# davidmilligan/MLVFS

Hardware: AMD Instinct MI355X
Metric: Mpix/s, 3584x1320 14-bit unpack+badpix+cs5x5+stripes (fused, stream resident in HBM) (higher is better)
Workload: dtype u16/int32

## Files before the change

### mlvfs_amd/csrc/k_frame_p.hip

```cpp
#include "frame_plan.h"
#include "k_stream_dev.h"

namespace mlv {

constexpr int P_WAIT_MIN = 1, P_WAIT_MAX = 15;
template <bool SPREAD_>
struct __align__(16) SmemP {
    static constexpr bool SPREAD = SPREAD_;
    uint16_t raw[2 * RH][2 * TCW];
    uint32_t pk[PH][PW];
    int ge[RH][TCW];
    uint16_t t16[MLV_T16_N + (SPREAD_ ? 64 : 0)];
    uint32_t has_patch[PMAP_WORDS];
    uint32_t xchg[3][XCHG_WORDS];
    int unc[2];
    int low[2];
    int dim[2];
    int next_tile, next_end;
    int walk[5];
    int2 carry_at[256];
    uint4 carry_spare;
};

struct PGroup {
    mlv_pk16 s[4][5];
    mlv_pk16 p0[10], p1[10];
    mlv_pk16 q[6];
};
struct PNext { mlv_pk16 s0[5], s2[5], p0[10], q[6]; };

__device__ __forceinline__ mlv_pk16 as_pk(uint32_t v) { return __builtin_bit_cast(mlv_pk16, v); }
__device__ __forceinline__ uint32_t as_u(mlv_pk16 v) { return __builtin_bit_cast(uint32_t, v); }

__device__ __forceinline__ void pchain_group(const uint32_t (*pk)[PW], int row_top, int col_left, PGroup &g)
{
    mlv_pk16 col[4][5];
#pragma unroll
    for (int r = 0; r < 5; r++) {
        const uint4 v = *(const uint4 *)&pk[row_top + r][col_left];
        col[0][r] = as_pk(v.x); col[1][r] = as_pk(v.y); col[2][r] = as_pk(v.z); col[3][r] = as_pk(v.w);
    }
#pragma unroll
    for (int c = 0; c < 4; c++) mlv_sort5(col[c], g.s[c]);
    mlv_merge55(g.s[0], g.s[1], g.p0);
    mlv_merge55(g.s[2], g.s[3], g.p1);
}
__device__ __forceinline__ void pchain_fetch_lists(const PGroup &g, PNext &n)
{
#pragma unroll
    for (int i = 0; i < 5; i++) { n.s0[i] = dpp_next(g.s[0][i]); n.s2[i] = dpp_next(g.s[2][i]); }
#pragma unroll
    for (int i = 0; i < 10; i++) n.p0[i] = dpp_next(g.p0[i]);
}
__device__ __forceinline__ void pchain_fetch_window(const PGroup &g, PNext &n)
{
#pragma unroll
    for (int i = 0; i < 6; i++) n.q[i] = dpp_next(g.q[i]);
}
__device__ __forceinline__ void pchain_publish(const PGroup &g, uint32_t *x)
{
    uint4 *o = (uint4 *)x;
    o[0] = make_uint4(as_u(g.s[0][0]), as_u(g.s[0][1]), as_u(g.s[0][2]), as_u(g.s[0][3]));
    o[1] = make_uint4(as_u(g.s[0][4]), as_u(g.s[2][0]), as_u(g.s[2][1]), as_u(g.s[2][2]));
    o[2] = make_uint4(as_u(g.s[2][3]), as_u(g.s[2][4]), as_u(g.p0[0]), as_u(g.p0[1]));
    o[3] = make_uint4(as_u(g.p0[2]), as_u(g.p0[3]), as_u(g.p0[4]), as_u(g.p0[5]));
    o[4] = make_uint4(as_u(g.p0[6]), as_u(g.p0[7]), as_u(g.p0[8]), as_u(g.p0[9]));
    o[5] = make_uint4(as_u(g.q[0]), as_u(g.q[1]), as_u(g.q[2]), as_u(g.q[3]));
    *(uint2 *)&o[6] = make_uint2(as_u(g.q[4]), as_u(g.q[5]));
}
__device__ __forceinline__ void pchain_collect_lists(const uint32_t *x, PNext &n)
{
    const uint4 *o = (const uint4 *)x;
    const uint4 a0 = o[0], a1 = o[1], a2 = o[2], a3 = o[3], a4 = o[4];
    n.s0[0] = as_pk(a0.x); n.s0[1] = as_pk(a0.y); n.s0[2] = as_pk(a0.z); n.s0[3] = as_pk(a0.w); n.s0[4] = as_pk(a1.x);
    n.s2[0] = as_pk(a1.y); n.s2[1] = as_pk(a1.z); n.s2[2] = as_pk(a1.w); n.s2[3] = as_pk(a2.x); n.s2[4] = as_pk(a2.y);
    n.p0[0] = as_pk(a2.z); n.p0[1] = as_pk(a2.w); n.p0[2] = as_pk(a3.x); n.p0[3] = as_pk(a3.y); n.p0[4] = as_pk(a3.z);
    n.p0[5] = as_pk(a3.w); n.p0[6] = as_pk(a4.x); n.p0[7] = as_pk(a4.y); n.p0[8] = as_pk(a4.z); n.p0[9] = as_pk(a4.w);
}
__device__ __forceinline__ void pchain_collect_window(const uint32_t *x, PNext &n)
{
    const uint4 a5 = *(const uint4 *)(x + 20);
    const uint2 a6 = *(const uint2 *)(x + 24);
    n.q[0] = as_pk(a5.x); n.q[1] = as_pk(a5.y); n.q[2] = as_pk(a5.z); n.q[3] = as_pk(a5.w); n.q[4] = as_pk(a6.x); n.q[5] = as_pk(a6.y);
}
__device__ __forceinline__ void pchain_finish(const PGroup &g, const PNext &n, mlv_pk16 (&o)[STRIP])
{
    mlv_pk16 q1[6], t[1];
    mlv_quad_mid6(g.p1, n.p0, q1);
    mlv_final6of11(g.q, n.s0, t);  o[0] = t[0];
    mlv_final6of11(q1, g.s[1], t); o[1] = t[0];
    mlv_final6of11(q1, n.s2, t);   o[2] = t[0];
    mlv_final6of11(n.q, g.s[3], t); o[3] = t[0];
}
__device__ __forceinline__ bool pk_uncertain(const mlv_pk16 (&o)[STRIP])
{
    typedef unsigned short upk16 __attribute__((ext_vector_type(2)));
    const upk16 off = { 32769, 32769 }, two = { 2, 2 };
    upk16 m = __builtin_bit_cast(upk16, o[0]) + off;
#pragma unroll
    for (int c = 1; c < STRIP; c++) m = __builtin_elementwise_min(m, (upk16)(__builtin_bit_cast(upk16, o[c]) + off));
    return __builtin_bit_cast(uint32_t, __builtin_elementwise_min(m, two)) != 0x00020002u;
}

__device__ __forceinline__ uint32_t add3_u32(uint32_t a, uint32_t b, uint32_t c)
{
    uint32_t r;
    asm("v_add3_u32 %0, %1, %2, %3" : "=v"(r) : "v"(a), "v"(b), "v"(c));
    return r;
}
template <int NC, bool SPREAD>
__device__ __forceinline__ void cell_multi_pk_fast(const uint32_t *p0, const uint32_t *p1, int black, const uint16_t *t, int ref_r, int ref_b,
                                                   int (&ge)[NC], uint32_t (&pk)[NC])
{
    uint32_t fb[4 * NC], tv[4 * NC];
    const float fmagic = 8388608.0f + (float)black;
#pragma unroll
    for (int c = 0; c < NC; c++) {
        const uint32_t px[4] = { p0[2 * c], p0[2 * c + 1], p1[2 * c], p1[2 * c + 1] };
#pragma unroll
        for (int i = 0; i < 4; i++) fb[4 * c + i] = __float_as_uint(__uint_as_float(px[i] | 0x4B000000u) - fmagic);
    }
#pragma unroll
    for (int i = 0; i < 4 * NC; i++) tv[i] = *(const uint16_t *)((const char *)t + t16_offset<SPREAD>(fb[i]));
    uint32_t exr[NC], exb[NC], exg[NC];
#pragma unroll
    for (int c = 0; c < NC; c++) { exr[c] = fb[4 * c] >> 8; exb[c] = fb[4 * c + 3] >> 8; exg[c] = (fb[4 * c + 1] + fb[4 * c + 2]) >> 8; }
#pragma unroll
    for (int c = 0; c < NC; c += 2) {
        asm volatile("" :: "v"(exr[c]), "v"(exb[c]), "v"(exg[c]), "v"(exr[c + 1]), "v"(exb[c + 1]), "v"(exg[c + 1]));
    }
#pragma unroll
    for (int i = 0; i < 4 * NC; i += 8) {
        asm volatile("" :: "v"(tv[i]), "v"(tv[i + 1]), "v"(tv[i + 2]), "v"(tv[i + 3]), "v"(tv[i + 4]), "v"(tv[i + 5]), "v"(tv[i + 6]), "v"(tv[i + 7]));
    }
    uint32_t nref_r = 0u - (uint32_t)ref_r, nref_b = 0u - (uint32_t)ref_b;
    asm("" : "+v"(nref_r), "+v"(nref_b));
#pragma unroll
    for (int c = 0; c < NC; c++) {
        const uint32_t gb = add3_u32(exg[c], tv[4 * c + 1], tv[4 * c + 2]) >> 1;
        ge[c] = (int)(gb - (127u << 15));
        uint32_t ngr = nref_r - gb, ngb = nref_b - gb;
        pk[c] = as_u(__builtin_amdgcn_cvt_pk_i16((int)add3_u32(exr[c], tv[4 * c + 0], ngr), (int)add3_u32(exb[c], tv[4 * c + 3], ngb)));
    }
}

template <int NC>
__device__ __forceinline__ void cell_multi_pk_tab(const uint32_t *p0, const uint32_t *p1, uint32_t koff, const int *tab, int ref_r, int ref_b,
                                                  int (&ge)[NC], uint32_t (&pk)[NC])
{
    uint32_t ev[4 * NC];
#pragma unroll
    for (int c = 0; c < NC; c++) {
        const uint32_t px[4] = { p0[2 * c], p0[2 * c + 1], p1[2 * c], p1[2 * c + 1] };
#pragma unroll
        for (int i = 0; i < 4; i++) ev[4 * c + i] = *(const uint32_t *)((const char *)tab + ((px[i] << 2) + koff));
    }
#pragma unroll
    for (int i = 0; i < 4 * NC; i += 8) {
        asm volatile("" :: "v"(ev[i]), "v"(ev[i + 1]), "v"(ev[i + 2]), "v"(ev[i + 3]), "v"(ev[i + 4]), "v"(ev[i + 5]), "v"(ev[i + 6]), "v"(ev[i + 7]));
    }
    uint32_t nref_r = 1u - (uint32_t)ref_r, nref_b = 1u - (uint32_t)ref_b;
    asm("" : "+v"(nref_r), "+v"(nref_b));
#pragma unroll
    for (int c = 0; c < NC; c++) {
        const uint32_t gb = (ev[4 * c + 1] + ev[4 * c + 2]) >> 1;
        ge[c] = (int)gb;
        const uint32_t ng = ~gb;
        pk[c] = as_u(__builtin_amdgcn_cvt_pk_i16((int)add3_u32(ev[4 * c + 0], nref_r, ng), (int)add3_u32(ev[4 * c + 3], nref_b, ng)));
    }
}
template <int NC>
__device__ __forceinline__ void cell_multi_pk_tab_dark(const uint32_t *p0, const uint32_t *p1, uint32_t koff, const int *tab, int ref_r, int ref_b,
                                                       int (&ge)[NC], uint32_t (&pk)[NC])
{
    int ev[4 * NC];
#pragma unroll
    for (int c = 0; c < NC; c++) {
        const uint32_t px[4] = { p0[2 * c], p0[2 * c + 1], p1[2 * c], p1[2 * c + 1] };
#pragma unroll
        for (int i = 0; i < 4; i++) ev[4 * c + i] = *(const int *)((const char *)tab + max((int)((px[i] << 2) + koff), 0));
    }
#pragma unroll
    for (int i = 0; i < 4 * NC; i += 8) {
        asm volatile("" :: "v"(ev[i]), "v"(ev[i + 1]), "v"(ev[i + 2]), "v"(ev[i + 3]), "v"(ev[i + 4]), "v"(ev[i + 5]), "v"(ev[i + 6]), "v"(ev[i + 7]));
    }
#pragma unroll
    for (int c = 0; c < NC; c++) {
        ge[c] = half_trunc(wadd(ev[4 * c + 1], ev[4 * c + 2]));
        const int dr = wsub(ev[4 * c + 0], ge[c]), db = wsub(ev[4 * c + 3], ge[c]);
        pk[c] = as_u(__builtin_amdgcn_cvt_pk_i16(__builtin_elementwise_sub_sat(dr, ref_r), __builtin_elementwise_sub_sat(db, ref_b)));
    }
}

template <class SM>
__device__ __forceinline__ void emit_item_p(SM &sm, int black, bool dark, bool slow, int ref_r, int ref_b, int p, int lk, bool edge,
                                            const uint32_t (&p0)[8], const uint32_t (&p1)[8])
{
    const int jj = p - HC;
    const bool keep = !edge && jj >= 0;
    int ge[4];
    uint32_t pk[4];
    if (!dark) cell_multi_pk_fast<4, SM::SPREAD>(p0, p1, black, sm.t16, ref_r, ref_b, ge, pk);
    else {
        int dr[4], db[4];
#pragma unroll
        for (int c = 0; c < 4; c += 2) {
            int g2[2], r2[2], b2[2];
            if (!slow) cell_multi_ev_dark<2, SM::SPREAD>(p0 + 2 * c, p1 + 2 * c, black, sm.t16, g2, r2, b2);
            else cell_pair_ev<SM::SPREAD>(p0 + 2 * c, p1 + 2 * c, black, sm.t16, true, g2, r2, b2);
            ge[c] = g2[0]; ge[c + 1] = g2[1]; dr[c] = r2[0]; dr[c + 1] = r2[1]; db[c] = b2[0]; db[c + 1] = b2[1];
        }
#pragma unroll
        for (int c = 0; c < 4; c++)
            pk[c] = as_u(__builtin_amdgcn_cvt_pk_i16(__builtin_elementwise_sub_sat(dr[c], ref_r), __builtin_elementwise_sub_sat(db[c], ref_b)));
    }
    const int ca = edge ? PW - HC : HC + 4 * lk, cb = edge ? 0 : ca + 2;
    const uint32_t prow = __umul24((uint32_t)p, (uint32_t)(PW * 4));
    char *ppk = (char *)&sm.pk[0][0] + prow;
    *(uint2 *)(ppk + 4 * ca) = make_uint2(pk[0], pk[1]);
    *(uint2 *)(ppk + 4 * cb) = make_uint2(pk[2], pk[3]);
    if (keep) {
        *(int4 *)&sm.ge[jj][4 * lk] = make_int4(ge[0], ge[1], ge[2], ge[3]);
        *(uint4 *)&sm.raw[2 * jj][8 * lk] = make_uint4(p0[0] | (p0[1] << 16), p0[2] | (p0[3] << 16), p0[4] | (p0[5] << 16), p0[6] | (p0[7] << 16));
        *(uint4 *)&sm.raw[2 * jj + 1][8 * lk] = make_uint4(p1[0] | (p1[1] << 16), p1[2] | (p1[3] << 16), p1[4] | (p1[5] << 16), p1[6] | (p1[7] << 16));
    }
}

template <bool PACKED, int VEC, bool SPREAD>
__global__ __launch_bounds__(256, 4) void k_frame_p(const FrameArgs a)
{
    static_assert(VEC != 0, "rows of whole 8-pixel groups");
    constexpr int METHOD = 5;
    using Smem = SmemP<SPREAD>;
    __shared__ Smem sm;
    constexpr int BPP = bpp_of(PACKED, VEC);
    constexpr int NEW0 = 2 * HC;
    const int tid = threadIdx.x;

    load_t16_rel<SPREAD>(sm.t16, cold_args()->t16, tid);
    {
        constexpr int C_PL = 2 * HC * PW * 4 / 16, C_RAW = 2 * HC * 2 * TCW * 2 / 16, C_GE = HC * TCW * 4 / 16, C_ALL = C_PL + C_RAW + C_GE;
        static_assert(C_ALL <= 256, "one 16-byte piece per thread");
        int to = (int)offsetof(Smem, carry_spare), delta = 0;
        if (tid < C_PL) { to = (int)offsetof(Smem, pk) + 16 * tid; delta = TCH * PW * 4; }
        else if (tid < C_PL + C_RAW) { to = (int)offsetof(Smem, raw) + 16 * (tid - C_PL); delta = 2 * TCH * 2 * TCW * 2; }
        else if (tid < C_ALL) { to = (int)offsetof(Smem, ge) + 16 * (tid - C_PL - C_RAW); delta = TCH * TCW * 4; }
        sm.carry_at[tid] = make_int2(to + delta, to);
    }
    const int tiles_per_frame = a.tiles_x * a.tiles_y;
    const bool pmap_ok = tiles_per_frame <= PMAP_WORDS * 32;
    int band_end;
    {
        KArgs ka = cold_args();
        if (ka->patch && pmap_ok) {
            for (int i = tid; i < PMAP_WORDS; i += 256) sm.has_patch[i] = 0;
            __syncthreads();
            const int *toff = ka->tile_off;
            for (int i = tid; i < tiles_per_frame; i += 256)
                if (toff[i + 1] != toff[i]) atomicOr(&sm.has_patch[i >> 5], 1u << (i & 31));
        }
        const int total = tiles_per_frame * ka->nframes;
        const int groups = ka->groups, nx = 8;
        const int grp = blockIdx.x % groups;
        const int gpx = (groups + nx - 1) / nx;
        const int grank = (groups % nx == 0) ? (grp % nx) * gpx + grp / nx : grp;
        const int gq = total / groups, grem = total - gq * groups;
        const int band_start = grank * gq + min(grank, grem);
        band_end = band_start + gq + (grank < grem ? 1 : 0);
        const int run = max(ka->run, 1);
        const int runs_len = max(band_end - band_start - ka->singles, 0) / run * run;
        if (tid == 0) { sm.walk[0] = band_start; sm.walk[1] = runs_len; sm.walk[2] = run; sm.walk[3] = grp; sm.walk[4] = 0; }
    }
    auto draw = [&](int &nt, int &ne) {
        KArgs ka = cold_args();
        int *tickets = ka->tickets;
        const int band_start = sm.walk[0], runs_len = sm.walk[1], run = sm.walk[2], grp = sm.walk[3];
        if (!sm.walk[4]) {
            const int p = atomicAdd(&tickets[2 * grp], run);
            if (p < runs_len) { nt = band_start + p; ne = nt + run; return; }
            sm.walk[4] = 1;
        }
        const int q = atomicAdd(&tickets[2 * grp + 1], 1);
        nt = min(band_start + runs_len + q, band_end);
        ne = nt + 1;
    };
    if (tid == 0) {
        int nt, ne;
        draw(nt, ne);
        sm.next_tile = nt; sm.next_end = ne;
        sm.unc[0] = 0; sm.unc[1] = 0; sm.low[0] = 0; sm.low[1] = 0; sm.dim[0] = 0; sm.dim[1] = 0;
    }
    __syncthreads();
    int t = __builtin_amdgcn_readfirstlane(sm.next_tile), t_end = __builtin_amdgcn_readfirstlane(sm.next_end);
    struct Pos { int f, tcol, trow; };
    auto pos_of = [&](int tt) {
        Pos p;
        p.f = tt / tiles_per_frame;
        const int r = tt - p.f * tiles_per_frame;
        p.tcol = r / a.tiles_y;
        p.trow = r - p.tcol * a.tiles_y;
        return p;
    };
    auto pos_below = [&](Pos p) {
        if (++p.trow == a.tiles_y) {
            p.trow = 0;
            if (++p.tcol == a.tiles_x) { p.tcol = 0; p.f++; }
        }
        return p;
    };
    uint32_t r0[4], r1[4];
    uint32_t pre_a, pre_b;
    {
        const bool e0 = tid >= N_MAIN;
        item_tile_offsets<BPP>(item_lane<PACKED, VEC>(tid & 15, e0), e0 ? tid - N_MAIN : tid >> 4, a.w, pre_a, pre_b);
    }
    struct Src { const uint8_t *p; size_t stride; unsigned bytes; };
    auto src_of = [](KArgs ka) { Src s; s.p = ka->src; s.stride = ka->src_stride; s.bytes = ka->src_bytes; return s; };
    auto issue_tile = [&](const Src &sa, const Pos &p, int tl) {
        issue_tile_rows_pre<BPP, VEC>(r0, r1, sa.p + (size_t)p.f * sa.stride, sa.bytes, pre_a, pre_b,
                                      [&](int &row) { const bool l_edge = tl >= N_MAIN; row = l_edge ? tl - N_MAIN : tl >> 4; return item_lane<PACKED, VEC>(tl & 15, l_edge); },
                                      a.w, a.h, p.tcol * 2 * TCW, p.trow * 2 * TCH, NEW0);
    };
    uint32_t smp = 0, smp_sh = 0;
    auto issue_sample = [&](const Src &sa, const Pos &p, int tl) {
        const uint8_t *frame = sa.p + (size_t)p.f * sa.stride;
        const int x0 = min(p.tcol * 2 * TCW + TCW, (a.w - 16) & ~1), y0 = min(p.trow * 2 * TCH + TCH - 1, (a.h - 4) & ~1);
        const uint32_t i = (uint32_t)(y0 + ((tl >> 4) & 3)) * (uint32_t)a.w + (uint32_t)(x0 + (tl & 15));
        if (BPP != 16) {
            const uint32_t bit = i * (uint32_t)BPP;
            __builtin_memcpy(&smp, frame + 2 * (bit >> 4), 4);
            smp_sh = bit & 15u;
        } else smp = ((const uint16_t *)frame)[i];
    };
    int ref_r = 0, ref_b = 0;
    auto take_sample = [&]() {
        uint32_t px = smp;
        if (BPP != 16) px = (__builtin_amdgcn_alignbit(smp, smp, 16) >> (32 - BPP - smp_sh)) & ((1u << BPP) - 1u);
        const int l = min(max((int)px - a.black, 1), 16383);
        const int ix = ev_index(l);
        const int ev = ev_value(l, (int)sm.t16[SPREAD ? ix + (ix >> 7) : ix]);
        constexpr int CX[5] = { 0, 3, 6, 1, 5 }, CY[5] = { 0, 0, 0, 1, 1 };
        int dr[5], db[5];
#pragma unroll
        for (int c = 0; c < 5; c++) {
            constexpr int dummy = 0; (void)dummy;
            const int l0 = 2 * CX[c] + 32 * CY[c];
            const int r = __builtin_amdgcn_readlane(ev, l0), g1 = __builtin_amdgcn_readlane(ev, l0 + 1);
            const int g2 = __builtin_amdgcn_readlane(ev, l0 + 16), b = __builtin_amdgcn_readlane(ev, l0 + 17);
            const int ge = (g1 + g2) >> 1;
            dr[c] = r - ge; db[c] = b - ge;
        }
        auto med5 = [](const int (&v)[5]) { return med3i(v[4], max(min(v[0], v[1]), min(v[2], v[3])), min(max(v[0], v[1]), max(v[2], v[3]))); };
        ref_r = med5(dr);
        ref_b = med5(db);
    };
    Pos cur = pos_of(min(t, max(band_end - 1, 0)));
    {
        const Src sa = src_of(cold_args());
        issue_tile(sa, cur, tid);
        issue_sample(sa, cur, tid);
    }
    __syncthreads();

    int fb_skip = 0, fb_wait = P_WAIT_MIN;
    bool cont = false;
    int par = 0;
    int low_prev = 3;
    bool have_smp = true;
    auto push = [&](int first, int n) {
        KArgs ka = cold_args();
        int *ctl = ka->wl_ctl;
        const int i = atomicAdd(&ctl[0], 1);
        ka->wl[i] = make_int2(first, n);
        atomicAdd(&ctl[3], n);
    };
    while (t < band_end) {
        if (fb_skip > 0) {
            const int n = min(fb_skip, t_end - t);
            fb_skip -= n;
            if (tid == 0) {
                push(t, n);
                int nt, ne;
                if (t + n < t_end) { nt = t + n; ne = t_end; }
                else draw(nt, ne);
                sm.next_tile = nt; sm.next_end = ne;
            }
            lds_barrier();
            t = __builtin_amdgcn_readfirstlane(sm.next_tile); t_end = __builtin_amdgcn_readfirstlane(sm.next_end);
            lds_barrier();
            cont = false;
            if (t < band_end) {
                cur = pos_of(t);
                const Src sa = src_of(cold_args());
                issue_tile(sa, cur, tid);
                issue_sample(sa, cur, tid);
                have_smp = true;
            }
            continue;
        }
        int nt = 0, ne = 0;
        if (tid == 0) {
            if (t + 1 < t_end) { nt = t + 1; ne = t_end; }
            else draw(nt, ne);
        }
        const int trow = cur.trow, tx0 = cur.tcol * 2 * TCW, ty0 = cur.trow * 2 * TCH;
        const int tr = cur.trow * a.tiles_x + cur.tcol;
        const Src sa = src_of(cold_args());
        bool tile_patched = false;
        int pbeg = 0, pend = 0;
        int4 my_rec = make_int4(-1, 0, 0, 0);
        if (a.patch) {
            tile_patched = !pmap_ok || ((sm.has_patch[tr >> 5] >> (tr & 31)) & 1u);
            if (tile_patched) {
                KArgs ka = cold_args();
                const int *toff = ka->tile_off;
                pbeg = toff[tr];
                pend = toff[tr + 1];
                if (pbeg + tid < pend) my_rec = (ka->cells + (size_t)cur.f * ka->n_rec)[pbeg + tid];
            }
        }
        __builtin_amdgcn_s_setprio(0);
        if (!cont) {
            if (!have_smp) issue_sample(sa, cur, tid);
            take_sample();
        }
        int tid_o = tid;
        asm volatile("" : "+v"(tid_o));
        auto do_item = [&](const ItemLane &L, const uint32_t (&d0)[4], const uint32_t (&d1)[4], int p, int lk) {
            uint32_t p0[8], p1[8];
            unpack8<BPP>(d0, L.s0, L.s1, L.s23, p0);
            unpack8<BPP>(d1, L.s0 ^ L.flip, L.s1 ^ L.flip, L.s23 ^ L.flip, p1);
            uint32_t lo = min(p0[0], p1[0]), hi = max(p0[0], p1[0]);
#pragma unroll
            for (int i = 1; i < 8; i++) {
                lo = min(min(lo, p0[i]), p1[i]);
                if (!PACKED) hi = max(max(hi, p0[i]), p1[i]);
            }
            const bool odd = (int)lo <= a.black;
            const bool beyond = (!PACKED && (int)hi - a.black > 16383) || (PACKED && a.black < 0);
            const bool slow = (!PACKED || a.black < 0) && __any(beyond);
            const bool dark = slow || __any(odd);
            if (__any((int)lo <= a.black + 255) || slow) {
                sm.dim[par] = 1;
                if (__any((int)lo <= a.black + 64)) sm.low[par] = 1;
            }
            emit_item_p<Smem>(sm, a.black, dark, slow, ref_r, ref_b, p, lk, L.edge, p0, p1);
        };
        if (!cont) {
            if (tid_o < N_TOP) {
                const bool te = tid_o >= N_TOP_MAIN;
                const int trw = te ? tid_o - N_TOP_MAIN : tid_o >> 4;
                const ItemLane TL = item_lane<PACKED, VEC>(tid_o & 15, te);
                uint32_t q0[4] = { 0, 0, 0, 0 }, q1[4] = { 0, 0, 0, 0 };
                issue_item<BPP, true>(q0, q1, frame_rsrc(sa.p + (size_t)cur.f * sa.stride, sa.bytes), TL, a.w, a.h, tx0, ty0, trw);
                do_item(TL, q0, q1, trw, tid_o & 15);
            }
        }
        if (tid_o < N_ITEMS) {
            const bool l_edge = tid_o >= N_MAIN;
            do_item(item_lane<PACKED, VEC>(tid_o & 15, l_edge), r0, r1, NEW0 + (l_edge ? tid_o - N_MAIN : tid_o >> 4), tid_o & 15);
        }
        if (tid == 0) { sm.next_tile = nt; sm.next_end = ne; }
        lds_barrier();
        if (tid == 0) { sm.unc[par ^ 1] = 0; sm.low[par ^ 1] = 0; sm.dim[par ^ 1] = 0; }
        const int low_cur = tile_patched ? 3 : (__builtin_amdgcn_readfirstlane(sm.low[par]) | __builtin_amdgcn_readfirstlane(sm.dim[par]) << 1);
        const int t_next = __builtin_amdgcn_readfirstlane(sm.next_tile), t_end_next = __builtin_amdgcn_readfirstlane(sm.next_end);
        const bool cont_next = t_next == t + 1 && trow + 1 < a.tiles_y && t_next < band_end;
        if (tile_patched) {
            KArgs ka = cold_args();
            const int4 *cells = ka->cells + (size_t)cur.f * ka->n_rec;
            auto patch_one = [&](int4 rec) {
                PatchCell c = patch_cell<METHOD, PACKED, Smem>(sm, a.black, rec, tx0, ty0);
                if (c.i < 0) return;
                sm.pk[c.j][c.i] = as_u(__builtin_amdgcn_cvt_pk_i16(__builtin_elementwise_sub_sat(c.dr, ref_r), __builtin_elementwise_sub_sat(c.db, ref_b)));
                const int ii = c.i - HC, jj = c.j - HC;
                if (ii >= 0 && ii < TCW && jj >= 0 && jj < RH) {
                    sm.ge[jj][ii] = c.ge;
                    *(uint32_t *)&sm.raw[2 * jj][2 * ii] = c.top;
                    *(uint32_t *)&sm.raw[2 * jj + 1][2 * ii] = c.bot;
                }
            };
            patch_one(my_rec);
            for (int base = pbeg + 256; base < pend; base += 256)
                patch_one(base + tid < pend ? cells[base + tid] : make_int4(-1, 0, 0, 0));
            lds_barrier();
        }
        __builtin_amdgcn_s_setprio(1);
        Pos nxt = pos_below(cur);
        if (t_next != t + 1 || t_next >= band_end) nxt = pos_of(min(t_next, band_end - 1));
        {
            int tid_p = tid;
            asm volatile("" : "+v"(tid_p));
            issue_tile(sa, nxt, tid_p);
            if (!cont_next) issue_sample(sa, nxt, tid_p);
        }
        const OutArgs oa = out_args(cold_args());

        int tid_m = tid;
        asm volatile("" : "+v"(tid_m));
        const int j_ = (int)(__umul24((uint32_t)tid_m, 241u) >> 12);
        const int k = tid_m - (int)__umul24((uint32_t)j_, 17u);
        const int j = min(j_, TCH - 1);
        const bool is_strip = k < 16 && tid_m < 17 * TCH;
        const int y = ty0 + 2 * j;
        const bool smooth_row = y >= 4 && y < a.h - 5;
        mlv_pk16 o[STRIP] = { { 0, 0 }, { 0, 0 }, { 0, 0 }, { 0, 0 } };
        {
            const int lane = tid_m & 63;
            const bool publishes = lane == 0 && tid_m != 0, collects = lane == 63 && tid_m < 192;
            const int wv = tid_m >> 6;
            PGroup g;
            pchain_group(sm.pk, j, STRIP * k, g);
            mlv_quad_mid6(g.p0, g.p1, g.q);
            uint32_t *const xo = (uint32_t *)((char *)&sm.xchg[0][0] + __umul24((uint32_t)wv, (uint32_t)(XCHG_WORDS * 4)));
            if (publishes) pchain_publish(g, xo - XCHG_WORDS);
            lds_barrier();
            PNext n;
            pchain_fetch_lists(g, n);
            pchain_fetch_window(g, n);
            if (collects) { pchain_collect_lists(xo, n); pchain_collect_window(xo, n); }
            pchain_finish(g, n, o);
        }
        if (is_strip && smooth_row && pk_uncertain(o)) sm.unc[par] = 1;
        if (is_strip) {
            const int4 g4 = *(const int4 *)&sm.ge[j][STRIP * k];
            const int gev[STRIP] = { g4.x, g4.y, g4.z, g4.w };
            int er[STRIP], eb[STRIP];
#pragma unroll
            for (int c = 0; c < STRIP; c++) {
                er[c] = wadd(wadd(gev[c], ref_r), (int)o[c].x);
                eb[c] = wadd(wadd(gev[c], ref_b), (int)o[c].y);
            }
            strip_output<METHOD, PACKED, true, Smem>(sm, oa, a.w, a.h, a.black, cur.f, tx0, ty0, j, k, lanes_ge(y, 4) & lanes_lt(y, a.h - 5), gev, 0, er, eb, ((low_cur | low_prev) & 1) != 0, (low_cur | low_prev) == 0, true);
        }
        int4 carry = make_int4(0, 0, 0, 0);
        int2 c_at = make_int2(0, 0);
        if (cont_next) {
            c_at = sm.carry_at[tid];
            carry = *(const int4 *)((const char *)&sm + c_at.x);
        }
        lds_barrier();
        const int unc = __builtin_amdgcn_readfirstlane(sm.unc[par]);
        if (cont_next) *(int4 *)((char *)&sm + c_at.y) = carry;
        have_smp = !cont_next;
        if (unc) {
            if (tid == 0) push(t, 1);
            fb_skip = fb_wait;
            fb_wait = min(2 * fb_wait + 1, P_WAIT_MAX);
            cont = false;
        } else {
            fb_wait = P_WAIT_MIN;
            cont = cont_next;
        }
        low_prev = low_cur;
        t = t_next;
        t_end = t_end_next;
        cur = nxt;
        par ^= 1;
    }
    if (tid == 0) {
        KArgs ka = cold_args();
        const int groups = ka->groups;
        int *tickets = ka->tickets;
        if (atomicAdd(&tickets[2 * groups], 1) == (int)gridDim.x - 1)
            for (int i = 0; i <= 2 * groups; i++) tickets[i] = 0;
    }
}

template <bool SPREAD, int VEC>
__global__ __launch_bounds__(1024, 1) void k_frame_p5(const FrameArgs a, int cols, int segs, int seg_rows, int fold, int S_OUT)
{
    static_assert(!SPREAD, "one table layout");
    constexpr int BPP = 14;
    constexpr int WAVES = 16;
    constexpr int PARK_LANES = 62;
    struct __align__(16) Smem {
        int ev[MLV_EV32_N];
        uint4 park[WAVES][3][2][PARK_LANES];
    };
    static_assert(sizeof(Smem) <= 160 * 1024, "the CU's LDS");
    __shared__ Smem sm;
    {
        const uint4 *s4 = (const uint4 *)cold_args()->ev32;
        uint4 *d4 = (uint4 *)sm.ev;
        for (int i = (int)threadIdx.x; i < MLV_EV32_N * 4 / 16; i += 64 * WAVES) d4[i] = s4[i];
    }
    __syncthreads();
    const int lane = (int)threadIdx.x & 63;
    const int w = a.w, h = a.h, black = a.black;
    const uint32_t koff = 4u - 4u * (uint32_t)black;
    const int rows = h >> 1;
    const StreamGrid sg = stream_grid(cols, segs, fold);
    const int ntasks = cold_args()->nframes * sg.per_frame;
    const uint32_t pitch = (uint32_t)(w >> 3) * 14u;
    int *tickets = cold_args()->tickets;
    uint4 (*const mypark)[2][PARK_LANES] = sm.park[threadIdx.x >> 6];
    const int plane = min(max(lane - 1, 0), PARK_LANES - 1);
    const bool parks = lane >= 1 && lane <= PARK_LANES;
    for (;;) {
        const int task = stream_draw(tickets, lane);
        if (task >= ntasks) break;
        const StreamTask t = stream_task<VEC>(task, sg, segs, seg_rows, fold, S_OUT, lane, w, rows);
        const int f = t.f, c = t.c, j0 = t.j0, j1 = t.j1, nparts = t.nparts, P = t.P, roff = t.roff;
        KArgs kt = cold_args();
        const uint8_t *const frame = kt->src + (size_t)f * kt->src_stride;
        const mlv_i32x4 rs_in = frame_rsrc(frame, kt->src_bytes);
        const mlv_i32x4 rs_out = frame_rsrc(kt->dst + (size_t)f * kt->dst_stride, (uint32_t)w * (uint32_t)h * 2u);
        const int tx0 = 8 * (c * S_OUT - 1);
        const bool xm = c == 0 || 8 * (c * S_OUT + S_OUT) > w - 4;
        uint32_t dA0[4], dA1[4], dB0[4], dB1[4];
        auto issue = [&](int r, uint32_t (&d0)[4], uint32_t (&d1)[4]) { stream_issue(rs_in, r, roff, rows, pitch, t.gbyte, d0, d1); };
        issue(j0 - 2, dA0, dA1);
        issue(j0 - 1, dB0, dB1);
        int ref_r, ref_b;
        {
            const int x0 = min(max(8 * (c * S_OUT + S_OUT / 2), 0), (w - 16) & ~1), y0 = min(j0 + j1, (h - 4) & ~1) & ~1;
            const uint32_t px = fetch_clamped<BPP>(frame, w, h, x0 + (lane & 15), y0 + (lane >> 4));
            const int ev = sm.ev[1 + min(max((int)px - black, 1), 16383)];
            constexpr int CX[5] = { 0, 3, 6, 1, 5 }, CY[5] = { 0, 0, 0, 1, 1 };
            int sdr[5], sdb[5];
#pragma unroll
            for (int k = 0; k < 5; k++) {
                const int l0 = 2 * CX[k] + 32 * CY[k];
                const int rr = __builtin_amdgcn_readlane(ev, l0), g1 = __builtin_amdgcn_readlane(ev, l0 + 1);
                const int g2 = __builtin_amdgcn_readlane(ev, l0 + 16), bb = __builtin_amdgcn_readlane(ev, l0 + 17);
                const int gg = (g1 + g2) >> 1;
                sdr[k] = rr - gg; sdb[k] = bb - gg;
            }
            auto med5 = [](const int (&v)[5]) { return med3i(v[4], max(min(v[0], v[1]), min(v[2], v[3])), min(max(v[0], v[1]), max(v[2], v[3]))); };
            ref_r = med5(sdr);
            ref_b = med5(sdb);
        }
        int n_pm = 0, pm_cell = -1;
        uint32_t pm_top = 0, pm_bot = 0;
        bool list_all = false;
        if (kt->patch) {
            KArgs ka = kt;
            const int4 *cells = ka->cells + (size_t)f * ka->n_rec;
            const int *toff = ka->tile_off;
            const int tx_n = ka->tiles_x, ty_n = ka->tiles_y;
            const int cx_lo = 4 * (c * S_OUT - 1), cx_hi = cx_lo + 4 * P;
            const int tc0 = max(cx_lo - HC, 0) / TCW, tc1 = min((cx_hi - 1 + HC) / TCW, tx_n - 1);
            for (int q = 0; q < nparts; q++) {
                const int j0q = j0 + q * seg_rows, j1q = min(j0q + seg_rows, rows);
                if (j0q >= rows) break;
                const int cy_lo = j0q - 2, cy_hi = j1q + 2;
                const int tr0 = max(cy_lo, 0) / TCH, tr1 = min((cy_hi - 1) / TCH, ty_n - 1), ntr = tr1 - tr0 + 1;
                constexpr int MAXTR = 6;
                int my_lo = 0, my_hi = 0;
                if (lane < ntr && lane < MAXTR) { my_lo = toff[(tr0 + lane) * tx_n + tc0]; my_hi = toff[(tr0 + lane) * tx_n + tc1 + 1]; }
                if (ntr > MAXTR) list_all = true;
                int4 rec[MAXTR];
#pragma unroll
                for (int i = 0; i < MAXTR; i++) {
                    const int rb = __builtin_amdgcn_readlane(my_lo, i), re = __builtin_amdgcn_readlane(my_hi, i);
                    rec[i] = (i < ntr && rb + lane < re) ? cells[rb + lane] : make_int4(-1, 0, 0, 0);
                    if (i < ntr && re - rb > 64) list_all = true;
                }
#pragma unroll
                for (int i = 0; i < MAXTR; i++) {
                    const int rcx = rec[i].x & 0xFFFF, rcy = rec[i].x >> 16;
                    const bool in = rec[i].x >= 0 && rcx >= cx_lo && rcx < cx_hi && rcy >= cy_lo && rcy < cy_hi && rcy / TCH == tr0 + i;
                    unsigned long long m = __ballot(in);
                    while (m) {
                        const int src = __builtin_ctzll(m);
                        m &= m - 1;
                        if (n_pm < 64) {
                            const int vx = __builtin_amdgcn_readlane(rec[i].x, src), vy = __builtin_amdgcn_readlane(rec[i].y, src), vz = __builtin_amdgcn_readlane(rec[i].z, src);
                            const int at = (((vx >> 16) - q * seg_rows) << 16) | (4 * P * q + (vx & 0xFFFF) - cx_lo);
                            if (lane == n_pm) { pm_cell = at; pm_top = (uint32_t)vy; pm_bot = (uint32_t)vz; }
                            n_pm++;
                        } else list_all = true;
                    }
                }
            }
        }
        uint32_t pkr[5][4] = {};
        int ge2[4] = { 0, 0, 0, 0 }, ge1[4] = { 0, 0, 0, 0 };
        int fl1 = 3, fl2 = 3, fl3 = 3, fl4 = 3;
        unsigned long long unc_lanes = 0;
        int unc_r0 = 1 << 30, unc_r1 = -1;
        auto step = [&](int r, uint32_t (&d0)[4], uint32_t (&d1)[4]) {
            uint32_t p0[8], p1[8];
            unpack8<BPP>(d0, t.sel, t.sel, t.sel, p0);
            unpack8<BPP>(d1, t.sel1, t.sel1, t.sel1, p1);
            if (r + 2 <= j1 + 1) issue(r + 2, d0, d1);
            if (n_pm) {
                unsigned long long m = __ballot(lane < n_pm && (pm_cell >> 16) == r);
                while (m) {
                    const int src = __builtin_ctzll(m);
                    m &= m - 1;
                    const int cell = __builtin_amdgcn_readlane(pm_cell, src);
                    const uint32_t t_ = (uint32_t)__builtin_amdgcn_readlane((int)pm_top, src), b_ = (uint32_t)__builtin_amdgcn_readlane((int)pm_bot, src);
                    const int cxr = cell & 0xFFFF;
                    const bool mine = (cxr >> 2) == lane;
                    const int cc = cxr & 3;
#pragma unroll
                    for (int k = 0; k < 4; k++)
                        if (mine && cc == k) { p0[2 * k] = t_ & 0xFFFFu; p0[2 * k + 1] = t_ >> 16; p1[2 * k] = b_ & 0xFFFFu; p1[2 * k + 1] = b_ >> 16; }
                }
            }
            bool dark;
            const int fl0 = stream_row_low(p0, p1, black, dark);
            int ge[4];
            uint32_t pk[4];
            if (!dark) cell_multi_pk_tab<4>(p0, p1, koff, sm.ev, ref_r, ref_b, ge, pk);
            else cell_multi_pk_tab_dark<4>(p0, p1, koff, sm.ev, ref_r, ref_b, ge, pk);
            {
                uint4 (&slot)[2][PARK_LANES] = mypark[(unsigned)(r + 6) % 3u];
                if (parks) {
                    slot[0][plane] = make_uint4(p0[0] | (p0[1] << 16), p0[2] | (p0[3] << 16), p0[4] | (p0[5] << 16), p0[6] | (p0[7] << 16));
                    slot[1][plane] = make_uint4(p1[0] | (p1[1] << 16), p1[2] | (p1[3] << 16), p1[4] | (p1[5] << 16), p1[6] | (p1[7] << 16));
                }
            }
#pragma unroll
            for (int i = 0; i < 4; i++) { pkr[0][i] = pkr[1][i]; pkr[1][i] = pkr[2][i]; pkr[2][i] = pkr[3][i]; pkr[3][i] = pkr[4][i]; pkr[4][i] = pk[i]; }
            const int jr = r - 2, y = 2 * jr, yl = y + 2 * roff;
            if (jr >= j0 && jr < j1) {
                const unsigned long long msmooth = lanes_ge(yl, 4) & lanes_lt(yl, h - 5);
                const bool smooth_row = y + 2 * (nparts - 1) * seg_rows >= 4 && y < h - 5;
                mlv_pk16 o[STRIP] = { { 0, 0 }, { 0, 0 }, { 0, 0 }, { 0, 0 } };
                if (smooth_row) {
                    PGroup gq;
                    {
                        mlv_pk16 col[4][5];
#pragma unroll
                        for (int rr = 0; rr < 5; rr++)
#pragma unroll
                            for (int cc = 0; cc < 4; cc++) col[cc][rr] = as_pk(pkr[rr][cc]);
#pragma unroll
                        for (int cc = 0; cc < 4; cc++) mlv_sort5(col[cc], gq.s[cc]);
                        mlv_merge55(gq.s[0], gq.s[1], gq.p0);
                        mlv_merge55(gq.s[2], gq.s[3], gq.p1);
                    }
                    mlv_quad_mid6(gq.p0, gq.p1, gq.q);
                    PNext n;
                    pchain_fetch_lists(gq, n);
                    pchain_fetch_window(gq, n);
                    mlv_pk16 oc[STRIP];
                    pchain_finish(gq, n, oc);
                    o[0] = as_pk((uint32_t)dpp_prev_i((int)as_u(oc[2]))); o[1] = as_pk((uint32_t)dpp_prev_i((int)as_u(oc[3])));
                    o[2] = oc[0]; o[3] = oc[1];
                    const unsigned long long um = __ballot(t.writes && pk_uncertain(o)) & msmooth;
                    if (um) { unc_lanes |= um; unc_r0 = min(unc_r0, jr); unc_r1 = max(unc_r1, jr); }
                }
                int er[STRIP], eb[STRIP];
#pragma unroll
                for (int cc = 0; cc < STRIP; cc++) {
                    er[cc] = wadd(wadd(ge2[cc], ref_r), (int)o[cc].x);
                    eb[cc] = wadd(wadd(ge2[cc], ref_b), (int)o[cc].y);
                }
                uint32_t top[STRIP], bot[STRIP];
                {
                    const uint4 (&slot)[2][PARK_LANES] = mypark[(unsigned)(jr + 6) % 3u];
                    const uint4 t4 = slot[0][plane], b4 = slot[1][plane];
                    top[0] = t4.x; top[1] = t4.y; top[2] = t4.z; top[3] = t4.w;
                    bot[0] = b4.x; bot[1] = b4.y; bot[2] = b4.z; bot[3] = b4.w;
                }
                const OutArgs oa = out_args(cold_args());
                stream_output<5>(oa, t, tx0, xm, rs_out, w, h, black, jr, yl, msmooth, fl0 | fl1 | fl2 | fl3 | fl4, ge2, er, eb, top, bot);
            }
#pragma unroll
            for (int cc = 0; cc < 4; cc++) { ge2[cc] = ge1[cc]; ge1[cc] = ge[cc]; }
            fl4 = fl3; fl3 = fl2; fl2 = fl1; fl1 = fl0;
        };
        for (int r = j0 - 2; r <= j1 + 1; r += 2) {
            step(r, dA0, dA1);
            if (r + 1 <= j1 + 1) step(r + 1, dB0, dB1);
        }
        if (list_all) { unc_lanes = ~0ull; unc_r0 = j0; unc_r1 = j1 - 1; }
        if (unc_lanes && lane == 0) {
            KArgs kl = cold_args();
            const int tnx = kl->tiles_x, tny = kl->tiles_y;
            int *ctl = kl->wl_ctl;
            for (int q = 0; q < nparts; q++) {
                const unsigned long long mq = P == 64 ? unc_lanes : (unc_lanes >> (q * P)) & ((1ull << P) - 1);
                const int r0 = unc_r0 + q * seg_rows, r1 = min(unc_r1 + q * seg_rows, rows - 1);
                if (!mq || r0 >= rows) continue;
                const int l0 = __builtin_ctzll(mq), l1 = 63 - __builtin_clzll(mq);
                const int cx0 = max(4 * (c * S_OUT + l0 - 1), 0), cx1 = min(4 * (c * S_OUT + l1 - 1) + 3, w / 2 - 1);
                const int tc0 = cx0 / TCW, tc1 = min(cx1 / TCW, tnx - 1), tr0 = r0 / TCH, tr1 = min(r1 / TCH, tny - 1);
                for (int tc = tc0; tc <= tc1; tc++) {
                    const int i = atomicAdd(&ctl[0], 1);
                    kl->wl[i] = make_int2(f * tnx * tny + tc * tny + tr0, tr1 - tr0 + 1);
                    atomicAdd(&ctl[3], tr1 - tr0 + 1);
                }
            }
        }
    }
    stream_last_out(tickets, lane, WAVES, [] {});
}

void launch_frame_p(const FramePlan &pl, int method, bool packed, int vec, bool spread, hipStream_t stream, const FrameArgs &a)
{
#ifdef KFP_ONLY
    hipLaunchKernelGGL((k_frame_p<true, 1, false>), dim3(pl.first_grid), dim3(256), 0, stream, a);
#else
    with_layout(method, packed, vec, spread, [&](auto M, auto P, auto V, auto S) {
        if constexpr (M.value == 5 && P.value && (V.value == 1 || V.value == 2)) {
            if (pl.first == FirstKernel::p5) {
                hipLaunchKernelGGL((k_frame_p5<false, V.value>), dim3((pl.first_grid + 3) / 4), dim3(1024), 0, stream, a, pl.cols, pl.segs, pl.seg_rows,
                                   pl.fold, FRAME_STREAM_COLW);
                return;
            }
        }
        if constexpr (M.value == 5 && V.value != 0)
            hipLaunchKernelGGL((k_frame_p<P.value, V.value, S.value>), dim3(pl.first_grid), dim3(256), 0, stream, a);
    });
#endif
}

void preload_k_frame_p() { hipFuncAttributes fa; (void)hipFuncGetAttributes(&fa, (const void *)k_frame_p<true, 1, false>); (void)hipGetLastError(); }

}
```

### mlvfs_amd/csrc/k_stream_dev.h

```cpp
#pragma once
#include "k_frame_dev.h"

namespace mlv {

struct StreamGrid { int ncols_full, nfolded, per_frame; };
__device__ __forceinline__ StreamGrid stream_grid(int cols, int segs, int fold)
{
    StreamGrid sg;
    sg.ncols_full = fold > 1 ? cols - 1 : cols;
    sg.nfolded = fold > 1 ? (segs + fold - 1) / fold : 0;
    sg.per_frame = sg.ncols_full * segs + sg.nfolded;
    return sg;
}

__device__ __forceinline__ int stream_draw(int *tickets, int lane)
{
    int task = 0;
    if (lane == 0) task = atomicAdd(&tickets[0], 1);
    return __builtin_amdgcn_readfirstlane(task);
}

struct StreamTask {
    int f, c;
    int j0, j1;
    int nparts, P;
    int pl, part, roff;
    int g;
    bool writes;
    uint32_t gbyte;
    uint32_t sel, sel1;
};
template <int VEC>
__device__ __forceinline__ StreamTask stream_task(int task, const StreamGrid &sg, int segs, int seg_rows, int fold, int S_OUT, int lane, int w, int rows)
{
    StreamTask t;
    const int gmax = (w >> 3) - 1;
    t.f = task / sg.per_frame;
    const int rem = task - t.f * sg.per_frame;
    const bool folded = rem >= sg.ncols_full * segs;
    t.c = folded ? sg.ncols_full : rem / segs;
    const int seg = folded ? (rem - sg.ncols_full * segs) * fold : rem - t.c * segs;
    t.j0 = seg * seg_rows; t.j1 = min(t.j0 + seg_rows, rows);
    t.nparts = folded ? fold : 1; t.P = folded ? 64 / fold : 64;
    t.pl = lane & (t.P - 1); t.part = folded ? lane / t.P : 0;
    t.roff = t.part * seg_rows;
    const int g_true = t.c * S_OUT + t.pl - 1;
    t.g = min(max(g_true, 0), gmax);
    t.writes = t.pl >= 1 && t.pl <= min(S_OUT, t.P - 2) && g_true <= gmax && t.j0 + t.roff < rows;
    t.gbyte = (uint32_t)t.g * 14u;
    t.sel = (t.g & 1) ? SEL_MIS : SEL_SWAP;
    t.sel1 = VEC == 2 ? t.sel ^ (SEL_SWAP ^ SEL_MIS) : t.sel;
    return t;
}

__device__ __forceinline__ void stream_issue(mlv_i32x4 rs_in, int r, int roff, int rows, uint32_t pitch, uint32_t gbyte, uint32_t (&d0)[4], uint32_t (&d1)[4])
{
    const int rr = min(max(r + roff, 0), rows - 1);
    const uint32_t o0u = __umul24((uint32_t)(2 * rr), pitch) + gbyte, o0 = o0u & ~3u, o1 = (o0u + pitch) & ~3u;
    const mlv_u32x2 a0 = mlv_rbl_x2(rs_in, (int)o0, 0, AUX_DEFAULT), b0 = mlv_rbl_x2(rs_in, (int)o0 + 8, 0, AUX_DEFAULT);
    const mlv_u32x2 a1 = mlv_rbl_x2(rs_in, (int)o1, 0, AUX_DEFAULT), b1 = mlv_rbl_x2(rs_in, (int)o1 + 8, 0, AUX_DEFAULT);
    d0[0] = a0.x; d0[1] = a0.y; d0[2] = b0.x; d0[3] = b0.y;
    d1[0] = a1.x; d1[1] = a1.y; d1[2] = b1.x; d1[3] = b1.y;
}

__device__ __forceinline__ int stream_row_low(const uint32_t (&p0)[8], const uint32_t (&p1)[8], int black, bool &dark)
{
    uint32_t lo = min(p0[0], p1[0]);
#pragma unroll
    for (int i = 1; i < 8; i++) lo = min(min(lo, p0[i]), p1[i]);
    dark = __any((int)lo <= black);
    int fl = 0;
    if (__any((int)lo <= black + 255)) fl = __any((int)lo <= black + 64) ? 3 : 2;
    return fl;
}

template <int METHOD>
__device__ __forceinline__ void stream_output(const OutArgs &oa, const StreamTask &t, int tx0, bool xm, mlv_i32x4 rs_out, int w, int h, int black, int jr, int yl,
                                              unsigned long long msmooth, int fl, const int (&ge)[STRIP], const int (&er)[STRIP], const int (&eb)[STRIP],
                                              uint32_t (&top)[STRIP], uint32_t (&bot)[STRIP])
{
    fl |= oa.stripes && smoothed_low(er, eb) ? 1 : 0;
    auto out = [&](auto CLAMP, auto XM, auto BRIGHT) {
        strip_output_t<METHOD, true, true, CLAMP.value, XM.value, false, BRIGHT.value, NoSmem, true>(NoSmem(), oa, w, h, black, t.f, tx0, 0, jr, t.pl, msmooth,
                                                                                                     ge, 0, er, eb, false, top, bot);
    };
    constexpr std::true_type Y{};
    constexpr std::false_type N{};
    if (fl & 1) { if (xm) out(Y, Y, N); else out(Y, N, N); }
    else if (xm) out(N, Y, N);
    else if (fl == 0) out(N, N, Y);
    else out(N, N, N);
    if (t.writes) {
        const uint32_t vo = (__umul24((uint32_t)yl, (uint32_t)w) + (uint32_t)(8 * t.g)) * 2u;
        const mlv_u32x4 vt = { top[0], top[1], top[2], top[3] }, vb = { bot[0], bot[1], bot[2], bot[3] };
        mlv_rbs_x4(vt, rs_out, (int)vo, 0, 2);
        mlv_rbs_x4(vb, rs_out, (int)vo, w * 2, 2);
    }
}

template <class AFTER>
__device__ __forceinline__ void stream_last_out(int *tickets, int lane, int waves_per_wg, AFTER after)
{
    if (lane == 0) {
        const int nwaves = (int)gridDim.x * waves_per_wg;
        if (atomicAdd(&tickets[1], 1) == nwaves - 1) {
            tickets[0] = 0; tickets[1] = 0;
            after();
        }
    }
}

}
```

Measured before the change: 906,300.

## Split row loop into prologue/steady/epilogue phases and defer prefetch before stores

The per-row loop becomes three compile-time specialised phases: a warmup that only prefetches, a steady state that outputs and prefetches, and a tail that outputs with no prefetch. Runtime row-range checks are removed from the loop body. In the steady state the next-row buffer load is issued after the output computation, just before the stores, through a new hook in stream_output. Output resource setup and the stripe args are hoisted or loaded early, and asm barriers pin register liveness. This aims to shorten live ranges and branches and to reorder memory issue for better overlap, at the cost of larger code and fragile scheduling hints.

After: 943,000, median of 6. 4.1% higher.

```diff
diff --git a/mlvfs_amd/csrc/k_frame_p.hip b/mlvfs_amd/csrc/k_frame_p.hip
--- a/mlvfs_amd/csrc/k_frame_p.hip
+++ b/mlvfs_amd/csrc/k_frame_p.hip
@@ -571,6 +571,7 @@
 __global__ __launch_bounds__(1024, 1) void k_frame_p5(const FrameArgs a, int cols, int segs, int seg_rows, int fold, int S_OUT)
 {
     static_assert(!SPREAD, "one table layout");
+    asm volatile("" : "+s"(cols));
     constexpr int BPP = 14;
     constexpr int WAVES = 16;
     constexpr int PARK_LANES = 62;
@@ -605,9 +606,9 @@
         KArgs kt = cold_args();
         const uint8_t *const frame = kt->src + (size_t)f * kt->src_stride;
         const mlv_i32x4 rs_in = frame_rsrc(frame, kt->src_bytes);
-        const mlv_i32x4 rs_out = frame_rsrc(kt->dst + (size_t)f * kt->dst_stride, (uint32_t)w * (uint32_t)h * 2u);
-        const int tx0 = 8 * (c * S_OUT - 1);
-        const bool xm = c == 0 || 8 * (c * S_OUT + S_OUT) > w - 4;
+        mlv_i32x4 rs_out = { 0, 0, 0, 0 };
+        int tx0 = 0;
+        bool xm = false;
         uint32_t dA0[4], dA1[4], dB0[4], dB1[4];
         auto issue = [&](int r, uint32_t (&d0)[4], uint32_t (&d1)[4]) { stream_issue(rs_in, r, roff, rows, pitch, t.gbyte, d0, d1); };
         issue(j0 - 2, dA0, dA1);
@@ -680,11 +681,15 @@
         int fl1 = 3, fl2 = 3, fl3 = 3, fl4 = 3;
         unsigned long long unc_lanes = 0;
         int unc_r0 = 1 << 30, unc_r1 = -1;
-        auto step = [&](int r, uint32_t (&d0)[4], uint32_t (&d1)[4]) {
+        auto step = [&](auto OUT, auto PRE, int r, uint32_t (&d0)[4], uint32_t (&d1)[4], const uint32_t (&n0)[4], const uint32_t (&n1)[4]) {
             uint32_t p0[8], p1[8];
             unpack8<BPP>(d0, t.sel, t.sel, t.sel, p0);
             unpack8<BPP>(d1, t.sel1, t.sel1, t.sel1, p1);
-            if (r + 2 <= j1 + 1) issue(r + 2, d0, d1);
+#ifdef P5_AB_EARLY_PREFETCH
+            if constexpr (PRE.value) issue(r + 2, d0, d1);
+#else
+            if constexpr (PRE.value && !OUT.value) issue(r + 2, d0, d1);
+#endif
             if (n_pm) {
                 unsigned long long m = __ballot(lane < n_pm && (pm_cell >> 16) == r);
                 while (m) {
@@ -715,8 +720,13 @@
             }
 #pragma unroll
             for (int i = 0; i < 4; i++) { pkr[0][i] = pkr[1][i]; pkr[1][i] = pkr[2][i]; pkr[2][i] = pkr[3][i]; pkr[3][i] = pkr[4][i]; pkr[4][i] = pk[i]; }
-            const int jr = r - 2, y = 2 * jr, yl = y + 2 * roff;
-            if (jr >= j0 && jr < j1) {
+            if constexpr (OUT.value) {
+                const int jr = r - 2, y = 2 * jr, yl = y + 2 * roff;
+#ifndef P5_AB_LATE_OUTARGS
+                KArgs ke = cold_args();
+                const uint2 *const e2d_early = ke->e2d;
+                const int stripes_early = ke->stripes;
+#endif
                 const unsigned long long msmooth = lanes_ge(yl, 4) & lanes_lt(yl, h - 5);
                 const bool smooth_row = y + 2 * (nparts - 1) * seg_rows >= 4 && y < h - 5;
                 mlv_pk16 o[STRIP] = { { 0, 0 }, { 0, 0 }, { 0, 0 }, { 0, 0 } };
@@ -757,16 +767,51 @@
                     top[0] = t4.x; top[1] = t4.y; top[2] = t4.z; top[3] = t4.w;
                     bot[0] = b4.x; bot[1] = b4.y; bot[2] = b4.z; bot[3] = b4.w;
                 }
+#ifndef P5_AB_LATE_OUTARGS
+                OutArgs oa = out_args(cold_args());
+                oa.e2d = e2d_early; oa.stripes = stripes_early;
+#else
                 const OutArgs oa = out_args(cold_args());
-                stream_output<5>(oa, t, tx0, xm, rs_out, w, h, black, jr, yl, msmooth, fl0 | fl1 | fl2 | fl3 | fl4, ge2, er, eb, top, bot);
+#endif
+                stream_output<5>(oa, t, tx0, xm, rs_out, w, h, black, jr, yl, msmooth, fl0 | fl1 | fl2 | fl3 | fl4, ge2, er, eb, top, bot, [&] {
+#ifndef P5_AB_EARLY_PREFETCH
+                    if constexpr (PRE.value) {
+                        asm volatile("" :: "v"(n0[0]), "v"(n0[1]), "v"(n0[2]), "v"(n0[3]), "v"(n1[0]), "v"(n1[1]), "v"(n1[2]), "v"(n1[3]));
+                        issue(r + 2, d0, d1);
+                    }
+#endif
+                });
             }
 #pragma unroll
             for (int cc = 0; cc < 4; cc++) { ge2[cc] = ge1[cc]; ge1[cc] = ge[cc]; }
             fl4 = fl3; fl3 = fl2; fl2 = fl1; fl1 = fl0;
         };
-        for (int r = j0 - 2; r <= j1 + 1; r += 2) {
-            step(r, dA0, dA1);
-            if (r + 1 <= j1 + 1) step(r + 1, dB0, dB1);
+        constexpr std::true_type Y{};
+        constexpr std::false_type N{};
+        int r = j0 - 2;
+#pragma unroll 1
+        for (; r < j0 + 2; r += 2) {
+            step(N, Y, r, dA0, dA1, dB0, dB1);
+            step(N, Y, r + 1, dB0, dB1, dA0, dA1);
+        }
+        asm volatile("" :: "v"(dA0[0]), "v"(dA0[1]), "v"(dA0[2]), "v"(dA0[3]), "v"(dA1[0]), "v"(dA1[1]), "v"(dA1[2]), "v"(dA1[3]));
+        {
+            KArgs ko = cold_args();
+            rs_out = frame_rsrc(ko->dst + (size_t)f * ko->dst_stride, (uint32_t)w * (uint32_t)h * 2u);
+            tx0 = 8 * (c * S_OUT - 1);
+            xm = c == 0 || 8 * (c * S_OUT + S_OUT) > w - 4;
+        }
+#pragma unroll 1
+        for (; r < j1; r += 2) {
+            step(Y, Y, r, dA0, dA1, dB0, dB1);
+            step(Y, Y, r + 1, dB0, dB1, dA0, dA1);
+        }
+#pragma unroll 1
+        for (bool second = false; r <= j1 + 1; r++, second = true) {
+            uint32_t e0[4], e1[4];
+#pragma unroll
+            for (int i = 0; i < 4; i++) { e0[i] = second ? dB0[i] : dA0[i]; e1[i] = second ? dB1[i] : dA1[i]; }
+            step(Y, N, r, e0, e1, e0, e1);
         }
         if (list_all) { unc_lanes = ~0ull; unc_r0 = j0; unc_r1 = j1 - 1; }
         if (unc_lanes && lane == 0) {
diff --git a/mlvfs_amd/csrc/k_stream_dev.h b/mlvfs_amd/csrc/k_stream_dev.h
--- a/mlvfs_amd/csrc/k_stream_dev.h
+++ b/mlvfs_amd/csrc/k_stream_dev.h
@@ -74,10 +74,11 @@
     return fl;
 }
 
-template <int METHOD>
+struct StreamNoHook { __device__ __forceinline__ void operator()() const {} };
+template <int METHOD, class BEFORE_STORES = StreamNoHook>
 __device__ __forceinline__ void stream_output(const OutArgs &oa, const StreamTask &t, int tx0, bool xm, mlv_i32x4 rs_out, int w, int h, int black, int jr, int yl,
                                               unsigned long long msmooth, int fl, const int (&ge)[STRIP], const int (&er)[STRIP], const int (&eb)[STRIP],
-                                              uint32_t (&top)[STRIP], uint32_t (&bot)[STRIP])
+                                              uint32_t (&top)[STRIP], uint32_t (&bot)[STRIP], BEFORE_STORES before_stores = BEFORE_STORES())
 {
     fl |= oa.stripes && smoothed_low(er, eb) ? 1 : 0;
     auto out = [&](auto CLAMP, auto XM, auto BRIGHT) {
@@ -90,6 +91,7 @@
     else if (xm) out(N, Y, N);
     else if (fl == 0) out(N, N, Y);
     else out(N, N, N);
+    before_stores();
     if (t.writes) {
         const uint32_t vo = (__umul24((uint32_t)yl, (uint32_t)w) + (uint32_t)(8 * t.g)) * 2u;
         const mlv_u32x4 vt = { top[0], top[1], top[2], top[3] }, vb = { bot[0], bot[1], bot[2], bot[3] };
```
